# trifectatechfoundation/zlib-rs

Hardware: NVIDIA H100
Metric: deflate_level6_raw_input_throughput_silesia_small_tar (higher is better)
Workload: dtype u8

## Files before the change

### __graft_entry__.py

```python
import os
import subprocess
import sys

ROOT = os.path.dirname(os.path.abspath(__file__))
if ROOT not in sys.path:
    sys.path.insert(0, ROOT)
sys.path.insert(0, os.path.join(ROOT, "tests"))


def build():
    subprocess.check_call(["make", "-C", os.path.join(ROOT, "zlib_rs_b200", "csrc"), "-j8"])
    subprocess.check_call(["make", "-C", os.path.join(ROOT, "oracle")])
    subprocess.check_call(["make", "-C", os.path.join(ROOT, "oracle"), "ref"])
    subprocess.check_call(["make", "-C", os.path.join(ROOT, "tests", "hostmodel")])
    subprocess.check_call(["make", "-C", os.path.join(ROOT, "tests", "skipmodel")])
    subprocess.check_call(["make", "-C", os.path.join(ROOT, "tests", "shardmodel")])
    subprocess.check_call(["make", "-C", os.path.join(ROOT, "tests", "membermodel")])
    subprocess.check_call(["make", "-C", os.path.join(ROOT, "tests", "bgzfmodel")])
    subprocess.check_call(["make", "-C", os.path.join(ROOT, "tests", "batchmodel")])
    subprocess.check_call(["make", "-C", os.path.join(ROOT, "tests", "batchdictmodel")])
    subprocess.check_call(["make", "-C", os.path.join(ROOT, "tests", "batchdictsmodel")])
    subprocess.check_call(["make", "-C", os.path.join(ROOT, "tests", "batchparammodel")])
    subprocess.check_call(["make", "-C", os.path.join(ROOT, "tests", "indexmodel")])
    subprocess.check_call(["make", "-C", os.path.join(ROOT, "tests", "writerindexmodel")])
    subprocess.check_call(["make", "-C", os.path.join(ROOT, "tests", "flushmodel")])
    subprocess.check_call(["make", "-C", os.path.join(ROOT, "tests", "bgzfindexmodel")])
    subprocess.check_call(["make", "-C", os.path.join(ROOT, "tests", "c_client")])
    import zlib_rs_b200
    zlib_rs_b200.lib()


def smoke():
    import zlib
    import zlib_rs_b200 as Z
    import oracle_lib as O
    from corpus import synthetic_mix
    d = synthetic_mix(300000, seed=1)
    out = Z.compress2(d, 6)
    assert out == O.compress(d, 6)[1], "GPU deflate differs from the oracle"
    assert zlib.decompress(out) == d
    assert Z.uncompress(out, len(d)) == d
    assert Z.crc32(d) == O.crc32(d) and Z.adler32(d) == O.adler32(d)
    print("smoke ok: %d -> %d bytes, bit-exact vs oracle" % (len(d), len(out)))


if __name__ == "__main__":
    build()
    if len(sys.argv) > 1 and sys.argv[1] == "smoke":
        smoke()
```

### zlib_rs_b200/csrc/zb_huff.h

```cpp
#pragma once
#include "zb_core.h"

namespace zb {

constexpr int kLCodes = 286, kDCodes = 30, kBlCodes = 19, kHeapSize = 2 * kLCodes + 1;
constexpr int kMaxBits = 15, kMaxBlBits = 7, kEndBlock = 256;
constexpr uint32_t kHdrBytes = 640;

struct HuffTables {
    uint8_t length_code[256];
    uint8_t dist_code[512];
    uint16_t base_length[29];
    uint16_t base_dist[30];
    uint16_t sl_code[288];
    uint8_t sl_len[288];
    uint16_t sd_code[30];
};

ZB_HD uint32_t extra_lbits(uint32_t c) { return (c < 8 || c == 28) ? 0 : (c - 4) >> 2; }
ZB_HD uint32_t extra_dbits(uint32_t c) { return c < 4 ? 0 : (c - 2) >> 1; }
ZB_HD uint32_t extra_blbits(uint32_t c) { return c == 16 ? 2 : c == 17 ? 3 : c == 18 ? 7 : 0; }
ZB_HD uint32_t bl_order(uint32_t i)
{
    return i < 3 ? 16 + i : (i & 1) ? (i == 3 ? 0 : 8 - (i - 3) / 2) : 8 + (i - 4) / 2;
}
ZB_HD uint32_t bit_reverse(uint32_t code, int len)
{
    uint32_t r = 0;
    for (int i = 0; i < len; i++) { r = (r << 1) | (code & 1); code >>= 1; }
    return r;
}
ZB_HD uint32_t d_code(const HuffTables &t, uint32_t dist) { return t.dist_code[dist < 256 ? dist : 256 + (dist >> 7)]; }

ZB_HDN inline void init_tables(HuffTables &t)
{
    int length = 0, dist = 0, code;
    for (code = 0; code < 28; code++) {
        t.base_length[code] = (uint16_t)length;
        for (int n = 0; n < (1 << extra_lbits(code)); n++) t.length_code[length++] = (uint8_t)code;
    }
    t.length_code[length - 1] = 28;
    t.base_length[28] = 0;
    for (code = 0; code < 16; code++) {
        t.base_dist[code] = (uint16_t)dist;
        for (int n = 0; n < (1 << extra_dbits(code)); n++) t.dist_code[dist++] = (uint8_t)code;
    }
    dist >>= 7;
    for (; code < kDCodes; code++) {
        t.base_dist[code] = (uint16_t)(dist << 7);
        for (int n = 0; n < (1 << (extra_dbits(code) - 7)); n++) t.dist_code[256 + dist++] = (uint8_t)code;
    }
    uint16_t next_code[16];
    uint16_t bl_count[16] = {0};
    for (int n = 0; n < 288; n++) {
        t.sl_len[n] = n <= 143 ? 8 : n <= 255 ? 9 : n <= 279 ? 7 : 8;
        bl_count[t.sl_len[n]]++;
    }
    uint32_t c = 0;
    next_code[0] = 0;
    for (int b = 1; b <= 15; b++) { c = (c + bl_count[b - 1]) << 1; next_code[b] = (uint16_t)c; }
    for (int n = 0; n < 288; n++) t.sl_code[n] = (uint16_t)bit_reverse(next_code[t.sl_len[n]]++, t.sl_len[n]);
    for (int n = 0; n < kDCodes; n++) t.sd_code[n] = (uint16_t)bit_reverse((uint32_t)n, 5);
}

struct CtData { uint16_t fc, dl; };

struct TreeScratch {
    CtData ltree[kHeapSize], dtree[2 * kDCodes + 1], bltree[2 * kBlCodes + 1];
    uint32_t heap[kHeapSize];
    uint8_t depth[kHeapSize];
    uint64_t hk[kHeapSize];
};

struct TreeState { uint64_t opt_len, static_len; };

ZB_HD uint32_t freq_depth(const CtData *tree, const uint8_t *depth, uint32_t i) { return ((uint32_t)tree[i].fc << 8) | depth[i]; }

ZB_HDN inline void pqdownheap(TreeScratch &s, int heap_len, int k)
{
    const uint64_t v = s.hk[k], v_val = v >> 16;
    int j = k << 1;
    while (j <= heap_len) {
        uint64_t e = s.hk[j];
        if (j < heap_len) {
            const uint64_t e1 = s.hk[j + 1];
            if ((e1 >> 16) <= (e >> 16)) { j++; e = e1; }
        }
        if (v_val <= (e >> 16)) break;
        s.hk[k] = e;
        k = j;
        j <<= 1;
    }
    s.hk[k] = v;
}
ZB_HD uint64_t heap_entry(const CtData *tree, const uint8_t *depth, uint32_t node) { return ((uint64_t)freq_depth(tree, depth, node) << 16) | node; }

ZB_HDN inline int build_tree(const HuffTables &t, TreeScratch &s, TreeState &st, CtData *tree, int kind)
{
    const int elems = kind == 0 ? kLCodes : kind == 1 ? kDCodes : kBlCodes;
    const int max_length = kind == 2 ? kMaxBlBits : kMaxBits;
    int heap_len = 0, heap_max = kHeapSize, max_code = -1, n, node;
    for (n = 0; n < elems; n++) {
        if (tree[n].fc != 0) { s.heap[++heap_len] = (uint32_t)(max_code = n); s.depth[n] = 0; }
        else tree[n].dl = 0;
    }
    while (heap_len < 2) {
        node = max_code < 2 ? ++max_code : 0;
        s.heap[++heap_len] = (uint32_t)node;
        tree[node].fc = 1;
        s.depth[node] = 0;
        st.opt_len--;
        if (kind == 0) st.static_len -= t.sl_len[node];
        else if (kind == 1) st.static_len -= 5;
    }
    for (n = 1; n <= heap_len; n++) s.hk[n] = heap_entry(tree, s.depth, s.heap[n]);
    for (n = heap_len / 2; n >= 1; n--) pqdownheap(s, heap_len, n);
    node = elems;
    do {
        n = (int)(s.hk[1] & 0xffffu);
        s.hk[1] = s.hk[heap_len--];
        pqdownheap(s, heap_len, 1);
        int m = (int)(s.hk[1] & 0xffffu);
        s.heap[--heap_max] = (uint32_t)n;
        s.heap[--heap_max] = (uint32_t)m;
        tree[node].fc = (uint16_t)(tree[n].fc + tree[m].fc);
        s.depth[node] = (uint8_t)((s.depth[n] >= s.depth[m] ? s.depth[n] : s.depth[m]) + 1);
        tree[n].dl = tree[m].dl = (uint16_t)node;
        s.hk[1] = heap_entry(tree, s.depth, (uint32_t)node);
        node++;
        pqdownheap(s, heap_len, 1);
    } while (heap_len >= 2);
    s.heap[--heap_max] = (uint32_t)(s.hk[1] & 0xffffu);

    uint16_t bl_count[kMaxBits + 1];
    int bits, h, overflow = 0;
    for (bits = 0; bits <= kMaxBits; bits++) bl_count[bits] = 0;
    tree[s.heap[heap_max]].dl = 0;
    for (h = heap_max + 1; h < kHeapSize; h++) {
        n = (int)s.heap[h];
        bits = tree[tree[n].dl].dl + 1;
        if (bits > max_length) { bits = max_length; overflow++; }
        tree[n].dl = (uint16_t)bits;
        if (n > max_code) continue;
        bl_count[bits]++;
        uint32_t xbits = kind == 0 ? (n >= 257 ? extra_lbits(n - 257) : 0) : kind == 1 ? extra_dbits(n) : extra_blbits(n);
        uint64_t f = tree[n].fc;
        st.opt_len += f * (uint64_t)(bits + xbits);
        if (kind == 0) st.static_len += f * (uint64_t)(t.sl_len[n] + xbits);
        else if (kind == 1) st.static_len += f * (uint64_t)(5 + xbits);
    }
    if (overflow > 0) {
        do {
            bits = max_length - 1;
            while (bl_count[bits] == 0) bits--;
// ... 9 lines not shown
                int m = (int)s.heap[--h];
                if (m > max_code) continue;
                if (tree[m].dl != (uint16_t)bits) {
                    st.opt_len += (uint64_t)bits * tree[m].fc;
                    st.opt_len -= (uint64_t)tree[m].dl * tree[m].fc;
                    tree[m].dl = (uint16_t)bits;
                }
                n--;
            }
        }
    }
    uint16_t next_code[kMaxBits + 1];
    uint32_t code = 0;
    next_code[0] = 0;
    for (bits = 1; bits <= kMaxBits; bits++) { code = (code + bl_count[bits - 1]) << 1; next_code[bits] = (uint16_t)code; }
    for (n = 0; n <= max_code; n++) {
        int len = tree[n].dl;
        if (len == 0) continue;
        tree[n].fc = (uint16_t)bit_reverse(next_code[len]++, len);
    }
    return max_code;
}

ZB_HDN inline void scan_tree(CtData *bltree, CtData *tree, int max_code)
{
    int prevlen = -1, curlen, nextlen = tree[0].dl, count = 0, max_count = 7, min_count = 4;
    if (nextlen == 0) { max_count = 138; min_count = 3; }
    tree[max_code + 1].dl = 0xffff;
    for (int n = 0; n <= max_code; n++) {
        curlen = nextlen;
        nextlen = tree[n + 1].dl;
        if (++count < max_count && curlen == nextlen) continue;
        else if (count < min_count) bltree[curlen].fc += (uint16_t)count;
        else if (curlen != 0) {
            if (curlen != prevlen) bltree[curlen].fc++;
            bltree[16].fc++;
        } else if (count <= 10) bltree[17].fc++;
        else bltree[18].fc++;
        count = 0;
        prevlen = curlen;
        if (nextlen == 0) { max_count = 138; min_count = 3; }
        else if (curlen == nextlen) { max_count = 6; min_count = 3; }
        else { max_count = 7; min_count = 4; }
    }
}

struct BitSink {
    uint8_t *buf;
    uint32_t nbits;
    ZB_HD void put(uint32_t val, uint32_t len)
    {
        for (uint32_t i = 0; i < len; i++, nbits++) {
            if ((nbits & 7) == 0) buf[nbits >> 3] = 0;
            buf[nbits >> 3] |= (uint8_t)(((val >> i) & 1u) << (nbits & 7));
        }
    }
};

ZB_HDN inline void send_tree(BitSink &o, const CtData *bltree, const CtData *tree, int max_code)
{
    int prevlen = -1, curlen, nextlen = tree[0].dl, count = 0, max_count = 7, min_count = 4;
    if (nextlen == 0) { max_count = 138; min_count = 3; }
    for (int n = 0; n <= max_code; n++) {
        curlen = nextlen;
        nextlen = tree[n + 1].dl;
        if (++count < max_count && curlen == nextlen) continue;
        else if (count < min_count) { do { o.put(bltree[curlen].fc, bltree[curlen].dl); } while (--count != 0); }
        else if (curlen != 0) {
            if (curlen != prevlen) { o.put(bltree[curlen].fc, bltree[curlen].dl); count--; }
            o.put(bltree[16].fc, bltree[16].dl);
            o.put((uint32_t)(count - 3), 2);
        } else if (count <= 10) {
            o.put(bltree[17].fc, bltree[17].dl);
            o.put((uint32_t)(count - 3), 3);
        } else {
            o.put(bltree[18].fc, bltree[18].dl);
            o.put((uint32_t)(count - 11), 7);
        }
        count = 0;
        prevlen = curlen;
        if (nextlen == 0) { max_count = 138; min_count = 3; }
        else if (curlen == nextlen) { max_count = 6; min_count = 3; }
        else { max_count = 7; min_count = 4; }
    }
}

struct BlockDesc {
    uint32_t sym_begin, sym_count;
    uint32_t in_start, in_len;
    uint32_t type;
    uint32_t last;
    uint32_t hdr_bits;
    uint32_t data_type;
    uint32_t have_window;
    uint32_t no_eob;
    uint64_t body_bits;
    uint64_t bit_base;
    uint16_t lcode[kLCodes];
    uint8_t llen[kLCodes];
    uint16_t dcode[kDCodes];
    uint8_t dlen[kDCodes];
    uint8_t hdr[kHdrBytes];
};

ZB_HDN inline uint32_t detect_data_type(const uint32_t *lfreq)
{
    uint64_t mask = 0xf3ffc07fULL;
    for (int n = 0; n < 32; n++, mask >>= 1)
        if ((mask & 1) && lfreq[n] != 0) return 0;
    if (lfreq[9] != 0 || lfreq[10] != 0 || lfreq[13] != 0) return 1;
    for (int n = 32; n < 256; n++)
        if (lfreq[n] != 0) return 1;
    return 0;
}

ZB_HDN inline void build_block(const HuffTables &t, TreeScratch &s, BlockDesc &b, const uint32_t *lfreq, const uint32_t *dfreq,
                               bool have_window, bool strategy_fixed)
{
    uint64_t opt_lenb, static_lenb;
    int max_blindex = 0, lmax = 0, dmax = 0;
    TreeState st{0, 0};
    b.data_type = 2;
    b.no_eob = 0;
    if (b.sym_count == 0) {
        opt_lenb = static_lenb = 0;
        st.static_len = 7;
    } else {
        b.data_type = detect_data_type(lfreq);
        for (int n = 0; n < kHeapSize; n++) s.ltree[n] = CtData{(uint16_t)(n < kLCodes ? lfreq[n] : 0), 0};
        s.ltree[kEndBlock].fc = 1;
        for (int n = 0; n < 2 * kDCodes + 1; n++) s.dtree[n] = CtData{(uint16_t)(n < kDCodes ? dfreq[n] : 0), 0};
        for (int n = 0; n < 2 * kBlCodes + 1; n++) s.bltree[n] = CtData{0, 0};
        lmax = build_tree(t, s, st, s.ltree, 0);
        dmax = build_tree(t, s, st, s.dtree, 1);
        scan_tree(s.bltree, s.ltree, lmax);
        scan_tree(s.bltree, s.dtree, dmax);
        build_tree(t, s, st, s.bltree, 2);
        for (max_blindex = kBlCodes - 1; max_blindex >= 3; max_blindex--)
            if (s.bltree[bl_order(max_blindex)].dl != 0) break;
        st.opt_len += 3 * ((uint64_t)max_blindex + 1) + 5 + 5 + 4;
        opt_lenb = (st.opt_len + 3 + 7) >> 3;
        static_lenb = (st.static_len + 3 + 7) >> 3;
        if (static_lenb <= opt_lenb || strategy_fixed) opt_lenb = static_lenb;
    }
    BitSink o{b.hdr, 0};
    if ((uint64_t)b.in_len + 4 <= opt_lenb && have_window) {
        b.type = 0;
        o.put(b.last, 3);
        b.hdr_bits = 3;
        b.body_bits = 0;
    } else if (static_lenb == opt_lenb) {
        b.type = 1;
        o.put(2 | b.last, 3);
        b.hdr_bits = 3;
        b.body_bits = st.static_len;
        for (int n = 0; n < kLCodes; n++) { b.lcode[n] = t.sl_code[n]; b.llen[n] = t.sl_len[n]; }
        for (int n = 0; n < kDCodes; n++) { b.dcode[n] = t.sd_code[n]; b.dlen[n] = 5; }
    } else {
        b.type = 2;
        o.put(4 | b.last, 3);
        int lcodes = lmax + 1, dcodes = dmax + 1, blcodes = max_blindex + 1;
        o.put((uint32_t)(lcodes - 257), 5);
        o.put((uint32_t)(dcodes - 1), 5);
        o.put((uint32_t)(blcodes - 4), 4);
        for (int r = 0; r < blcodes; r++) o.put(s.bltree[bl_order(r)].dl, 3);
        send_tree(o, s.bltree, s.ltree, lcodes - 1);
// ... 53 lines not shown
```

### zlib_rs_b200/csrc/zb_kernels.cu

```cuda
#include "zb_kernels.cuh"

namespace zb {

__constant__ HuffTables c_tab;

cudaError_t upload_tables()
{
    HuffTables t;
    init_tables(t);
    return cudaMemcpyToSymbol(c_tab, &t, sizeof t);
}

struct GAcc {
    const uint8_t *data;
    uint32_t N;
    const uint16_t *L;
    const uint32_t *holes;
    const uint32_t *M;
    uint32_t w = kWSize;
    __device__ __forceinline__ uint32_t byte(uint32_t y) const
    {
        while (y >= N) {
            if (y < 2 * w) return 0;
            y -= w;
        }
        return data[y];
    }
    __device__ __forceinline__ uint32_t link(uint32_t y) const { return y + 4 <= N ? L[y] : 0; }
    __device__ __forceinline__ bool inserted(uint32_t y) const { return !((holes[y >> 5] >> (y & 31)) & 1u); }
    __device__ __forceinline__ Match mlook(uint32_t x) const
    {
        uint32_t v = M[x];
        return Match{v >> 16, x - (v & 0xffffu)};
    }
};

struct SAcc {
    const uint8_t *sdata;
    const uint16_t *sL;
    const uint32_t *sholes;
    uint32_t ws;
    __device__ __forceinline__ uint32_t byte(uint32_t y) const { return sdata[y - ws]; }
    __device__ __forceinline__ uint32_t link(uint32_t y) const { return sL[y - ws]; }
    __device__ __forceinline__ bool inserted(uint32_t y) const
    {
        uint32_t i = y - ws;
        return !((sholes[i >> 5] >> (i & 31)) & 1u);
    }
};

struct SAccR {
    const uint8_t *sdata;
    const uint16_t *sL;
    uint32_t ws;
    __device__ __forceinline__ uint32_t byte(uint32_t y) const { return sdata[y - ws]; }
    __device__ __forceinline__ uint32_t link(uint32_t y) const { const uint32_t v = sL[y - ws]; return v == 0xffffu ? 0u : v; }
    __device__ __forceinline__ bool inserted(uint32_t) const { return true; }
};


__device__ __forceinline__ uint32_t lds_u32(const uint32_t *words, uint32_t byte_idx)
{
    const uint32_t w = byte_idx >> 2;
    return __funnelshift_r(words[w], words[w + 1], (byte_idx & 3u) * 8u);
}

constexpr uint32_t kFirstFlag = 0xffffu;

template <bool kRoll>
__device__ __forceinline__ void links2_body(const JobBufs &jb, uint32_t tile0)
{
    const uint32_t tile = tile0 + blockIdx.x;
    extern __shared__ __align__(16) uint8_t smem[];
    constexpr uint32_t kKeys = kRoll ? 32768u : 65536u;
    uint16_t *head = reinterpret_cast<uint16_t *>(smem);
    uint16_t *lists = reinterpret_cast<uint16_t *>(smem + kKeys * 2);
    uint8_t *sd = smem + kKeys * 2 + kLinkTile * 2;
    uint16_t *run = reinterpret_cast<uint16_t *>(smem + kKeys * 2 + kLinkTile * 2 + kLinkTile + 64);
    __shared__ uint16_t c_base[32], c_total[32];
    const uint32_t *words = reinterpret_cast<const uint32_t *>(sd);
    const uint32_t tid = threadIdx.x, lane = tid & 31, warp = tid >> 5;
    const uint32_t N = jb.N, need = kRoll ? 3u : 4u, cap = kRoll ? jb.wsize - 1u : jb.wsize - kMinLookahead;
    const uint32_t ts = tile * kLinkTile;
// ... 1083 lines not shown
};

__global__ void __launch_bounds__(32) k_tail(JobBufs jb)
{
    __shared__ uint32_t ins[1024];
    if (threadIdx.x != 0) return;
    GAcc a{jb.in, jb.N, jb.L, jb.holes, jb.M, jb.wsize};
    const uint32_t p0 = max(jb.info->tail_entry, jb.start);
    const uint32_t n_mid = jb.info->n_mid_syms;
    uint32_t k = 0;
    Sym *syms = jb.syms + n_mid;
    uint32_t *sb = jb.sym_base;
    if (jb.N - p0 > 1024u * 32u - 64u) { atomicOr(&jb.info->error, 4u); return; }
    auto emit = [&](const Sym &s, uint32_t B) {
        syms[k] = s;
        sb[k] = B;
        k++;
    };
    uint32_t fb;
    if (jb.wsize == kWSize) fb = serial_medium(a, jb.N, p0, ins, 1024u, jb.lp, emit);
    else fb = serial_medium(GAccW{a, jb.wsize}, jb.N, p0, ins, 1024u, jb.lp, emit, DynWin{jb.wsize});
    jb.info->n_syms = n_mid + k;
    jb.info->final_base = fb;
    jb.info->n_blocks = (n_mid + k) / jb.block_syms + 1;
}

__device__ __forceinline__ uint32_t sym_end(const Sym &s) { return s.pos + (s.dist ? (uint32_t)s.lc + 3u : 1u); }

__device__ __forceinline__ void block_hist_body(const Sym *syms, uint32_t begin, uint32_t count, uint32_t *fb)
{
    __shared__ uint32_t lf[kLCodes], df[kDCodes];
    for (uint32_t i = threadIdx.x; i < kLCodes; i += blockDim.x) lf[i] = 0;
    if (threadIdx.x < kDCodes) df[threadIdx.x] = 0;
    __syncthreads();
    for (uint32_t i = threadIdx.x; i < count; i += blockDim.x) {
        const Sym s = syms[begin + i];
        if (s.dist == 0) atomicAdd(&lf[s.lc], 1u);
        else {
            atomicAdd(&lf[257 + c_tab.length_code[s.lc]], 1u);
            atomicAdd(&df[d_code(c_tab, s.dist - 1u)], 1u);
        }
    }
    __syncthreads();
    for (uint32_t i = threadIdx.x; i < kLCodes; i += blockDim.x) fb[i] = lf[i];
    if (threadIdx.x < kDCodes) fb[kLCodes + threadIdx.x] = df[threadIdx.x];
}

__global__ void __launch_bounds__(256) k_block_hist(JobBufs jb, uint32_t *freq )
{
    const uint32_t b = blockIdx.x;
    const uint32_t nsyms = jb.info->n_syms, nblocks = jb.info->n_blocks;
    const uint32_t begin = b * jb.block_syms;
    const uint32_t count = (b + 1 < nblocks) ? jb.block_syms : nsyms - begin;
    block_hist_body(jb.syms, begin, count, freq + b * 320);
    if (threadIdx.x == 0) {
        BlockDesc &bd = jb.blocks[b];
        const bool last = b + 1 == nblocks;
        bd.sym_begin = begin;
        bd.sym_count = count;
        bd.last = last && !jb.not_last;
        const uint32_t start = begin == 0 ? jb.start : sym_end(jb.syms[begin - 1]);
        const uint32_t end = last ? jb.N : sym_end(jb.syms[begin + count - 1]);
        bd.in_start = start;
        bd.in_len = end - start;
        uint32_t Bf;
        if (last) Bf = jb.info->final_base;
        else {
            const uint32_t li = begin + count - 1, n_mid = jb.info->n_mid_syms;
            if (jb.serial_mode) {
                Bf = jb.serial_mode == 2 ? jb.block_base[b] : 0;
            } else if (jb.huffman_only) {
                const uint32_t q = jb.syms[li].pos, w = jb.wsize;
                Bf = q < 2 * w ? 0 : w * (1 + (q - 2 * w) / w);
            } else if (jb.slow_mode == 2) {
                Bf = base_at(jb.syms[li].pos, jb.N, jb.wsize);
            } else if (jb.slow_mode) {
                Bf = base_at(jb.syms[li].pos + 1, jb.N, jb.wsize);
            } else Bf = li < n_mid ? wbase_w(DynWin{jb.wsize}, jb.syms[li].pos) : jb.sym_base[li - n_mid];
        }
        bd.have_window = start >= Bf;
    }
}

__device__ __forceinline__ uint32_t brev_bits(uint32_t code, uint32_t len) { return __brev(code) >> (32u - len); }

template <int KIND>
__device__ __forceinline__ uint32_t xbits_of(uint32_t n) { return KIND == 0 ? (n >= 257 ? extra_lbits(n - 257) : 0u) : KIND == 1 ? extra_dbits(n) : extra_blbits(n); }

template <int KIND>
__device__ int build_tree_warp(TreeScratch &s, TreeState &st, CtData *tree, uint32_t *sh_cnt )
{
    constexpr int elems = KIND == 0 ? kLCodes : KIND == 1 ? kDCodes : kBlCodes;
    constexpr int max_length = KIND == 2 ? kMaxBlBits : kMaxBits;
    const uint32_t lane = threadIdx.x & 31;
    int heap_len = 0, max_code = -1;
    for (int b0 = 0; b0 < elems; b0 += 32) {
        const int n = b0 + (int)lane;
        const bool nz = n < elems && tree[n].fc != 0;
        const uint32_t m = __ballot_sync(0xffffffffu, nz);
        if (nz) { s.heap[heap_len + 1 + __popc(m & ((1u << lane) - 1u))] = (uint32_t)n; s.depth[n] = 0; }
        else if (n < elems) tree[n].dl = 0;
        heap_len += __popc(m);
        if (m) max_code = b0 + 31 - __clz(m);
    }
    __syncwarp();
    if (heap_len < 2) {
        if (lane == 0) {
            while (heap_len < 2) {
                const int node = max_code < 2 ? ++max_code : 0;
                s.heap[++heap_len] = (uint32_t)node;
                tree[node].fc = 1;
                s.depth[node] = 0;
                st.opt_len--;
                if (KIND == 0) st.static_len -= c_tab.sl_len[node];
                else if (KIND == 1) st.static_len -= 5;
            }
        }
        heap_len = 2;
        max_code = __shfl_sync(0xffffffffu, max_code, 0);
        __syncwarp();
    }
    for (int n = 1 + (int)lane; n <= heap_len; n += 32) s.hk[n] = heap_entry(tree, s.depth, s.heap[n]);
    __syncwarp();
    for (int lvl = 31 - __clz(heap_len / 2); lvl >= 0; lvl--) {
        const int first = 1 << lvl, last = min((2 << lvl) - 1, heap_len / 2);
        for (int k = first + (int)lane; k <= last; k += 32) pqdownheap(s, heap_len, k);
        __syncwarp();
    }
    int heap_max = kHeapSize;
    if (lane == 0) {
        int node = elems;
        do {
            const int n = (int)(s.hk[1] & 0xffffu);
            s.hk[1] = s.hk[heap_len--];
            pqdownheap(s, heap_len, 1);
            const int m = (int)(s.hk[1] & 0xffffu);
            s.heap[--heap_max] = (uint32_t)n;
            s.heap[--heap_max] = (uint32_t)m;
            tree[node].fc = (uint16_t)(tree[n].fc + tree[m].fc);
            s.depth[node] = (uint8_t)((s.depth[n] >= s.depth[m] ? s.depth[n] : s.depth[m]) + 1);
            tree[n].dl = tree[m].dl = (uint16_t)node;
            s.hk[1] = heap_entry(tree, s.depth, (uint32_t)node);
            node++;
            pqdownheap(s, heap_len, 1);
        } while (heap_len >= 2);
        s.heap[--heap_max] = (uint32_t)(s.hk[1] & 0xffffu);
        int overflow = 0;
        tree[s.heap[heap_max]].dl = 0;
        for (int h = heap_max + 1; h < kHeapSize; h++) {
            const int n = (int)s.heap[h];
            int bits = tree[tree[n].dl].dl + 1;
            if (bits > max_length) { bits = max_length; overflow++; }
            tree[n].dl = (uint16_t)bits;
        }
        sh_cnt[0] = (uint32_t)overflow;
    }
    heap_max = __shfl_sync(0xffffffffu, heap_max, 0);
    __syncwarp();
    const int overflow = (int)sh_cnt[0];
    __syncwarp();
    if (lane < 16) sh_cnt[lane] = 0;
    __syncwarp();
    uint64_t opt = 0, stat = 0;
    for (int n = (int)lane; n <= max_code; n += 32) {
        const uint32_t bits = tree[n].dl;
        if (tree[n].fc == 0 || bits == 0) continue;
        atomicAdd(&sh_cnt[bits], 1u);
        const uint32_t xb = xbits_of<KIND>((uint32_t)n);
        const uint64_t f = tree[n].fc;
        opt += f * (uint64_t)(bits + xb);
        if (KIND == 0) stat += f * (uint64_t)(c_tab.sl_len[n] + xb);
        else if (KIND == 1) stat += f * (uint64_t)(5 + xb);
    }
#pragma unroll
    for (int d = 16; d >= 1; d >>= 1) { opt += __shfl_xor_sync(0xffffffffu, opt, d); stat += __shfl_xor_sync(0xffffffffu, stat, d); }
    __syncwarp();
    if (lane == 0) {
        st.opt_len += opt;
        st.static_len += stat;
        if (overflow > 0) {
            int ov = overflow, bits;
            do {
                bits = max_length - 1;
                while (sh_cnt[bits] == 0) bits--;
                sh_cnt[bits]--;
                sh_cnt[bits + 1] += 2;
                sh_cnt[max_length]--;
                ov -= 2;
            } while (ov > 0);
            int h = kHeapSize;
            for (bits = max_length; bits != 0; bits--) {
                int n = (int)sh_cnt[bits];
                while (n != 0) {
                    const int m = (int)s.heap[--h];
                    if (m > max_code) continue;
                    if (tree[m].dl != (uint16_t)bits) {
                        st.opt_len += (uint64_t)bits * tree[m].fc;
                        st.opt_len -= (uint64_t)tree[m].dl * tree[m].fc;
                        tree[m].dl = (uint16_t)bits;
                    }
                    n--;
                }
            }
        }
    }
    __syncwarp();
    uint32_t nc = 0;
    {
        uint32_t code = 0;
        for (uint32_t b = 1; b <= (uint32_t)kMaxBits; b++) { code = (code + sh_cnt[b - 1]) << 1; if (b == lane) nc = code; }
    }
    for (int b0 = 0; b0 <= max_code; b0 += 32) {
        const int n = b0 + (int)lane;
        const uint32_t len = n <= max_code ? tree[n].dl : 0u;
        const uint32_t same = __match_any_sync(0xffffffffu, len);
        const uint32_t rank = __popc(same & ((1u << lane) - 1u));
        const uint32_t base = __shfl_sync(0xffffffffu, nc, len & 31u);
        if (len) tree[n].fc = (uint16_t)brev_bits(base + rank, len);
#pragma unroll 1
        for (uint32_t l = 1; l <= (uint32_t)kMaxBits; l++) {
            const uint32_t cnt = __popc(__ballot_sync(0xffffffffu, len == l));
            if (lane == l) nc += cnt;
        }
    }
    __syncwarp();
    return max_code;
}

struct WordSink {
    uint8_t *buf;
    uint32_t nbits;
    __device__ __forceinline__ void put(uint32_t val, uint32_t len)
    {
        const uint32_t byte = nbits >> 3, sh = nbits & 7u;
        const uint32_t v = (val & ((1u << len) - 1u)) << sh;
        if (sh == 0) buf[byte] = (uint8_t)v; else buf[byte] |= (uint8_t)v;
        if (sh + len > 8) { buf[byte + 1] = (uint8_t)(v >> 8); if (sh + len > 16) buf[byte + 2] = (uint8_t)(v >> 16); }
        nbits += len;
    }
};

__device__ void send_tree_fast(WordSink &o, const CtData *bltree, const CtData *tree, int max_code)
{
    int prevlen = -1, curlen, nextlen = tree[0].dl, count = 0, max_count = 7, min_count = 4;
    if (nextlen == 0) { max_count = 138; min_count = 3; }
    for (int n = 0; n <= max_code; n++) {
        curlen = nextlen;
        nextlen = tree[n + 1].dl;
        if (++count < max_count && curlen == nextlen) continue;
        else if (count < min_count) { do { o.put(bltree[curlen].fc, bltree[curlen].dl); } while (--count != 0); }
        else if (curlen != 0) {
            if (curlen != prevlen) { o.put(bltree[curlen].fc, bltree[curlen].dl); count--; }
            o.put(bltree[16].fc, bltree[16].dl);
            o.put((uint32_t)(count - 3), 2);
        } else if (count <= 10) {
            o.put(bltree[17].fc, bltree[17].dl);
            o.put((uint32_t)(count - 3), 3);
        } else {
            o.put(bltree[18].fc, bltree[18].dl);
            o.put((uint32_t)(count - 11), 7);
        }
        count = 0;
        prevlen = curlen;
        if (nextlen == 0) { max_count = 138; min_count = 3; }
        else if (curlen == nextlen) { max_count = 6; min_count = 3; }
        else { max_count = 7; min_count = 4; }
    }
}

__device__ void build_block_warp(TreeScratch &s, BlockDesc &b, const uint32_t *lfreq, const uint32_t *dfreq, bool have_window,
                                 bool strategy_fixed, uint32_t *sh_cnt, TreeState *sh_st)
{
    const uint32_t lane = threadIdx.x & 31;
    uint64_t opt_lenb = 0, static_lenb = 0;
    int max_blindex = 0, lmax = 0, dmax = 0;
    TreeState &st = *sh_st;
    if (lane == 0) { st = TreeState{0, 0}; b.data_type = 2; b.no_eob = 0; }
    __syncwarp();
    if (b.sym_count == 0) {
        if (lane == 0) st.static_len = 7;
    } else {
        {
            bool black = false, white = false;
            for (uint32_t n = lane; n < 256; n += 32) {
                if (lfreq[n] == 0) continue;
                if (n < 32 && ((0xf3ffc07fu >> n) & 1u)) black = true;
                if (n == 9 || n == 10 || n == 13 || n >= 32) white = true;
            }
            const bool ab = __any_sync(0xffffffffu, black), aw = __any_sync(0xffffffffu, white);
            if (lane == 0) b.data_type = ab ? 0u : aw ? 1u : 0u;
        }
        for (int n = (int)lane; n < kHeapSize; n += 32) s.ltree[n] = CtData{(uint16_t)(n < kLCodes ? lfreq[n] : 0), 0};
        for (int n = (int)lane; n < 2 * kDCodes + 1; n += 32) s.dtree[n] = CtData{(uint16_t)(n < kDCodes ? dfreq[n] : 0), 0};
        for (int n = (int)lane; n < 2 * kBlCodes + 1; n += 32) s.bltree[n] = CtData{0, 0};
        __syncwarp();
        if (lane == 0) s.ltree[kEndBlock].fc = 1;
        __syncwarp();
        lmax = build_tree_warp<0>(s, st, s.ltree, sh_cnt);
        dmax = build_tree_warp<1>(s, st, s.dtree, sh_cnt);
        if (lane == 0) {
            scan_tree(s.bltree, s.ltree, lmax);
            scan_tree(s.bltree, s.dtree, dmax);
        }
        __syncwarp();
        build_tree_warp<2>(s, st, s.bltree, sh_cnt);
        for (max_blindex = kBlCodes - 1; max_blindex >= 3; max_blindex--)
            if (s.bltree[bl_order(max_blindex)].dl != 0) break;
        if (lane == 0) st.opt_len += 3 * ((uint64_t)max_blindex + 1) + 5 + 5 + 4;
        __syncwarp();
        opt_lenb = (st.opt_len + 3 + 7) >> 3;
        static_lenb = (st.static_len + 3 + 7) >> 3;
        if (static_lenb <= opt_lenb || strategy_fixed) opt_lenb = static_lenb;
    }
    __syncwarp();
    if ((uint64_t)b.in_len + 4 <= opt_lenb && have_window) {
        if (lane == 0) { b.type = 0; b.hdr[0] = (uint8_t)b.last; b.hdr_bits = 3; b.body_bits = 0; }
    } else if (static_lenb == opt_lenb) {
        if (lane == 0) { b.type = 1; b.hdr[0] = (uint8_t)(2 | b.last); b.hdr_bits = 3; b.body_bits = st.static_len; }
        for (int n = (int)lane; n < kLCodes; n += 32) { b.lcode[n] = c_tab.sl_code[n]; b.llen[n] = c_tab.sl_len[n]; }
        if (lane < (uint32_t)kDCodes) { b.dcode[lane] = c_tab.sd_code[lane]; b.dlen[lane] = 5; }
    } else {
        if (lane == 0) {
            b.type = 2;
            WordSink o{b.hdr, 0};
            o.put(4 | b.last, 3);
            const int lcodes = lmax + 1, dcodes = dmax + 1, blcodes = max_blindex + 1;
            o.put((uint32_t)(lcodes - 257), 5);
            o.put((uint32_t)(dcodes - 1), 5);
            o.put((uint32_t)(blcodes - 4), 4);
            for (int r = 0; r < blcodes; r++) o.put(s.bltree[bl_order(r)].dl, 3);
            send_tree_fast(o, s.bltree, s.ltree, lcodes - 1);
            send_tree_fast(o, s.bltree, s.dtree, dcodes - 1);
            b.hdr_bits = o.nbits;
            b.body_bits = 3 + st.opt_len - o.nbits;
        }
        for (int n = (int)lane; n < kLCodes; n += 32) { b.lcode[n] = n <= lmax ? s.ltree[n].fc : 0; b.llen[n] = n <= lmax ? (uint8_t)s.ltree[n].dl : 0; }
        if (lane < (uint32_t)kDCodes) { b.dcode[lane] = (int)lane <= dmax ? s.dtree[lane].fc : 0; b.dlen[lane] = (int)lane <= dmax ? (uint8_t)s.dtree[lane].dl : 0; }
    }
    __syncwarp();
}

__device__ __forceinline__ void build_blocks_body(BlockDesc *gbd, const uint32_t *fb, bool quick, bool first, bool last_piece,
                                                  bool final_block, bool strategy_fixed)
{
    __shared__ TreeScratch s;
    __shared__ BlockDesc bd;
    __shared__ uint32_t fr[320];
    __shared__ uint32_t sh_cnt[16];
    __shared__ TreeState sh_st;
    for (uint32_t i = threadIdx.x; i < 320; i += 32) fr[i] = fb[i];
    for (uint32_t i = threadIdx.x; i < sizeof(BlockDesc) / 4; i += 32)
        reinterpret_cast<uint32_t *>(&bd)[i] = reinterpret_cast<const uint32_t *>(gbd)[i];
    __syncwarp();
    if (quick) {
        if (threadIdx.x == 0) build_quick_piece(c_tab, bd, fr, fr + kLCodes, first, last_piece, final_block);
    } else build_block_warp(s, bd, fr, fr + kLCodes, bd.have_window != 0, strategy_fixed, sh_cnt, &sh_st);
    __syncwarp();
    for (uint32_t i = threadIdx.x; i < sizeof(BlockDesc) / 4; i += 32)
        reinterpret_cast<uint32_t *>(gbd)[i] = reinterpret_cast<const uint32_t *>(&bd)[i];
}

__global__ void __launch_bounds__(32) k_build_blocks(JobBufs jb, const uint32_t *freq)
{
    const uint32_t b = blockIdx.x;
    if (b >= jb.info->n_blocks) return;
    build_blocks_body(&jb.blocks[b], freq + b * 320, jb.serial_mode == 1, b == 0, b + 1 == jb.info->n_blocks, jb.not_last == 0,
                      jb.strategy_fixed != 0);
}

__device__ __forceinline__ void or_bits(uint32_t *out32, uint64_t pos, uint64_t val, uint32_t n)
{
    if (n == 0) return;
    const uint64_t w = pos >> 5;
    const uint32_t sh = (uint32_t)(pos & 31);
    atomicOr(&out32[w], (uint32_t)(val << sh));
    if (sh + n > 32) {
        atomicOr(&out32[w + 1], (uint32_t)(val >> (32 - sh)));
        if (sh + n > 64) atomicOr(&out32[w + 2], (uint32_t)(val >> (64 - sh)));
    }
}

constexpr uint32_t kScanChunk = 1024;
__global__ void __launch_bounds__(256) k_scan_blocks(JobBufs jb)
{
    __shared__ uint64_t s_bits[kScanChunk];
    __shared__ uint64_t s_base[kScanChunk];
    __shared__ uint64_t s_bit;
    const uint32_t nb = jb.info->n_blocks;
    if (threadIdx.x == 0) s_bit = 8ull * jb.hdr_len + jb.prime_bits;
    for (uint32_t c0 = 0; c0 < nb; c0 += kScanChunk) {
        const uint32_t nc = min(kScanChunk, nb - c0);
        for (uint32_t i = threadIdx.x; i < nc; i += blockDim.x) {
            const BlockDesc &bd = jb.blocks[c0 + i];
            s_bits[i] = bd.type == 0 ? (1ull << 63) | (uint16_t)bd.in_len : (uint64_t)bd.hdr_bits + bd.body_bits;
        }
        __syncthreads();
        if (threadIdx.x == 0) {
            uint64_t bit = s_bit;
            for (uint32_t i = 0; i < nc; i++) {
                s_base[i] = bit;
                const uint64_t v = s_bits[i];
                bit = (v >> 63) ? ((bit + 3 + 7) & ~7ull) + 32 + 8ull * (v & 0xffffu) : bit + v;
            }
            s_bit = bit;
        }
        __syncthreads();
        for (uint32_t i = threadIdx.x; i < nc; i += blockDim.x) jb.blocks[c0 + i].bit_base = s_base[i];
        __syncthreads();
    }
    if (threadIdx.x != 0) return;
    uint64_t bit = s_bit;
    if (jb.not_last && jb.end_mode == 0) {
        const uint64_t p = (bit + 3 + 7) & ~7ull;
        jb.info->marker_byte = p >> 3;
        bit = p + 32;
    } else if (jb.not_last && jb.end_mode == 1) {
        or_bits(reinterpret_cast<uint32_t *>(jb.out), bit, 2u, 10);
        bit += 10;
    }
    jb.info->total_bits = bit;
    const uint64_t bytes = (jb.not_last && jb.end_mode ? (bit >> 3) : ((bit + 7) >> 3)) + (jb.wrap == 1 ? 4 : jb.wrap == 2 ? 8 : 0);
    jb.info->out_bytes = bytes;
    jb.info->data_type = jb.blocks[0].sym_count ? jb.blocks[0].data_type : 2u;
    if (bytes > jb.out_cap) { atomicOr(&jb.info->error, 8u); return; }
    stream_header(jb.out, jb.wrap, zlib_level_flags(jb.level, jb.huffman_only || jb.strategy_fixed), jb.cinfo, jb.xfl);
}

__device__ __forceinline__ void encode_body(const BlockDesc &bd, const Sym *syms, const uint8_t *in, uint8_t *out, uint32_t *error)
{
    __shared__ HuffTables st;
    __shared__ uint16_t s_lcode[kLCodes], s_dcode[kDCodes];
    __shared__ uint8_t s_llen[kLCodes], s_dlen[kDCodes];
    __shared__ uint64_t warp_sum[32];
    uint32_t *out32 = reinterpret_cast<uint32_t *>(out);
    const uint32_t tid = threadIdx.x;
    if (bd.type == 0) {
        const uint64_t p = ((bd.bit_base + 3 + 7) >> 3);
        const uint32_t sl = (uint16_t)bd.in_len;
        if (tid == 0) {
            or_bits(out32, bd.bit_base, bd.hdr[0] & 7u, 3);
            out[p] = (uint8_t)sl;
            out[p + 1] = (uint8_t)(sl >> 8);
// ... 308 lines not shown
```

Baseline: 1.648.

## Parallelize Huffman tree construction and header emission across the warp

Replaces the single-lane heap build with packed 32-bit or 64-bit heap keys and a vectorized sift-down. Bit lengths are now computed by a warp-parallel pointer-jumping pass instead of a serial walk. The run-length scan and tree header emission become warp-parallel, using ballot-found runs, a prefix sum of bit counts and atomicOr writes into a zeroed header. The goal is to shorten the serial latency of the per-block tree-building kernel, at the cost of extra shared memory, more synchronisation and new bit-exactness risks. Optional clock64 stamps for profiling are added behind a compile flag.

```diff
diff --git a/__graft_entry__.py b/__graft_entry__.py
--- a/__graft_entry__.py
+++ b/__graft_entry__.py
@@ -25,6 +25,7 @@
     subprocess.check_call(["make", "-C", os.path.join(ROOT, "tests", "writerindexmodel")])
     subprocess.check_call(["make", "-C", os.path.join(ROOT, "tests", "flushmodel")])
     subprocess.check_call(["make", "-C", os.path.join(ROOT, "tests", "bgzfindexmodel")])
+    subprocess.check_call(["make", "-C", os.path.join(ROOT, "tests", "huffmodel")])
     subprocess.check_call(["make", "-C", os.path.join(ROOT, "tests", "c_client")])
     import zlib_rs_b200
     zlib_rs_b200.lib()
diff --git a/zlib_rs_b200/csrc/zb_huff.h b/zlib_rs_b200/csrc/zb_huff.h
--- a/zlib_rs_b200/csrc/zb_huff.h
+++ b/zlib_rs_b200/csrc/zb_huff.h
@@ -69,7 +69,7 @@
     CtData ltree[kHeapSize], dtree[2 * kDCodes + 1], bltree[2 * kBlCodes + 1];
     uint32_t heap[kHeapSize];
     uint8_t depth[kHeapSize];
-    uint64_t hk[kHeapSize];
+    alignas(16) uint64_t hk[kHeapSize + 3];
 };
 
 struct TreeState { uint64_t opt_len, static_len; };
@@ -245,6 +245,25 @@
         if (nextlen == 0) { max_count = 138; min_count = 3; }
         else if (curlen == nextlen) { max_count = 6; min_count = 3; }
         else { max_count = 7; min_count = 4; }
+    }
+}
+
+template <class Emit>
+ZB_HDN inline void run_codes(uint32_t v, uint32_t len, Emit &&emit)
+{
+    uint32_t max_count = v == 0 ? 138u : 7u, min_count = v == 0 ? 3u : 4u;
+    bool first = true;
+    while (len) {
+        uint32_t count = len < max_count ? len : max_count;
+        len -= count;
+        if (count < min_count) { do emit(v, 0u, 0u); while (--count != 0); }
+        else if (v != 0) {
+            if (first) { emit(v, 0u, 0u); count--; }
+            emit(16u, count - 3, 2u);
+        } else if (count <= 10) emit(17u, count - 3, 3u);
+        else emit(18u, count - 11, 7u);
+        first = false;
+        if (v != 0) { max_count = 6; min_count = 3; }
     }
 }
 
diff --git a/zlib_rs_b200/csrc/zb_kernels.cu b/zlib_rs_b200/csrc/zb_kernels.cu
--- a/zlib_rs_b200/csrc/zb_kernels.cu
+++ b/zlib_rs_b200/csrc/zb_kernels.cu
@@ -1,4 +1,5 @@
 #include "zb_kernels.cuh"
+#include <cstdio>
 
 namespace zb {
 
@@ -1248,10 +1249,136 @@
     }
 }
 
+#ifdef ZB_BUILD_CYCLES
+__shared__ long long zb_stamp[12];
+#define ZB_STAMP(i) do { if ((threadIdx.x & 31) == 0) zb_stamp[i] = clock64(); } while (0)
+#else
+#define ZB_STAMP(i) do { } while (0)
+#endif
+
 __device__ __forceinline__ uint32_t brev_bits(uint32_t code, uint32_t len) { return __brev(code) >> (32u - len); }
 
 template <int KIND>
 __device__ __forceinline__ uint32_t xbits_of(uint32_t n) { return KIND == 0 ? (n >= 257 ? extra_lbits(n - 257) : 0u) : KIND == 1 ? extra_dbits(n) : extra_blbits(n); }
+
+template <typename T, int NB, int DB>
+struct HeapKey {
+    using type = T;
+    static constexpr int nb = NB, fb = NB + DB;
+    static constexpr T node_mask = (T(1) << NB) - 1, depth_mask = (T(1) << DB) - 1;
+    __device__ __forceinline__ static T make(uint32_t freq, uint32_t depth, uint32_t node) { return ((T)freq << (NB + DB)) | ((T)depth << NB) | node; }
+};
+using Key32 = HeapKey<uint32_t, 10, 5>;
+using Key64 = HeapKey<unsigned long long, 16, 8>;
+constexpr uint32_t kKey32MaxTotal = 1u << 17;
+
+template <typename T> struct Vec2;
+template <> struct Vec2<uint32_t> { using type = uint2; };
+template <> struct Vec2<unsigned long long> { using type = ulonglong2; };
+
+template <typename K, typename T = typename K::type>
+__device__ __forceinline__ void sift_down(T *h, int heap_len, int k, T v)
+{
+    using V = typename Vec2<T>::type;
+    constexpr int NB = K::nb;
+    const T vv = v >> NB;
+    int j = k << 1;
+    V c = *reinterpret_cast<const V *>(h + j);
+    while (j <= heap_len) {
+        const V g0 = reinterpret_cast<const V *>(h + 2 * j)[0], g1 = reinterpret_cast<const V *>(h + 2 * j)[1];
+        const bool right = j < heap_len && (c.y >> NB) <= (c.x >> NB);
+        const T e = right ? c.y : c.x;
+        if (vv <= (e >> NB)) break;
+        h[k] = e;
+        k = j + (int)right;
+        c = right ? g1 : g0;
+        j = k << 1;
+    }
+    h[k] = v;
+}
+
+template <typename K, typename T = typename K::type>
+__device__ int heap_build_warp(TreeScratch &s, CtData *tree, int heap_len, int node)
+{
+    constexpr int NB = K::nb, FB = K::fb;
+    const uint32_t lane = threadIdx.x & 31;
+    T *h = reinterpret_cast<T *>(s.hk);
+    for (int n = 1 + (int)lane; n <= heap_len; n += 32) { const uint32_t v = s.heap[n]; h[n] = K::make(tree[v].fc, 0, v); }
+    __syncwarp();
+    for (int lvl = 31 - __clz(heap_len / 2); lvl >= 0; lvl--) {
+        const int first = 1 << lvl, last = min((2 << lvl) - 1, heap_len / 2);
+        for (int k = first + (int)lane; k <= last; k += 32) sift_down<K>(h, heap_len, k, h[k]);
+        __syncwarp();
+    }
+    int heap_max = kHeapSize;
+    if (lane == 0) {
+        do {
+            const T kn = h[1];
+            sift_down<K>(h, heap_len - 1, 1, h[heap_len]);
+            heap_len--;
+            const T km = h[1];
+            const uint32_t n = (uint32_t)(kn & K::node_mask), m = (uint32_t)(km & K::node_mask);
+            s.heap[--heap_max] = n;
+            s.heap[--heap_max] = m;
+            const uint32_t f = (uint16_t)((uint32_t)(kn >> FB) + (uint32_t)(km >> FB));
+            const uint32_t dn = (uint32_t)((kn >> NB) & K::depth_mask), dm = (uint32_t)((km >> NB) & K::depth_mask);
+            tree[node].fc = (uint16_t)f;
+            tree[n].dl = tree[m].dl = (uint16_t)node;
+            sift_down<K>(h, heap_len, 1, K::make(f, (max(dn, dm) + 1) & (uint32_t)K::depth_mask, (uint32_t)node));
+            node++;
+        } while (heap_len >= 2);
+        s.heap[--heap_max] = (uint32_t)(h[1] & K::node_mask);
+    }
+    __syncwarp();
+    return __shfl_sync(0xffffffffu, heap_max, 0);
+}
+
+template <int MAX_LENGTH>
+__device__ int tree_lengths_warp(TreeScratch &s, CtData *tree, int heap_max)
+{
+    constexpr int kPer = (kHeapSize + 31) / 32;
+    const uint32_t lane = threadIdx.x & 31;
+    uint32_t *A = reinterpret_cast<uint32_t *>(s.hk), *B = A + kHeapSize + 3;
+    const uint32_t root = s.heap[heap_max];
+    uint32_t nd[kPer];
+#pragma unroll
+    for (int i = 0; i < kPer; i++) {
+        const int h = heap_max + (int)lane + 32 * i;
+        nd[i] = h < kHeapSize ? s.heap[h] : 0xffffu;
+        if (nd[i] != 0xffffu) A[nd[i]] = nd[i] == root ? root << 16 : ((uint32_t)tree[nd[i]].dl << 16) | 1u;
+    }
+    __syncwarp();
+    for (;;) {
+        bool more = false;
+#pragma unroll
+        for (int i = 0; i < kPer; i++) {
+            if (nd[i] == 0xffffu) continue;
+            uint32_t w = A[nd[i]];
+            const uint32_t p = w >> 16;
+            if (p != root) {
+                const uint32_t wp = A[p];
+                w = (wp & 0xffff0000u) | ((w & 0xffffu) + (wp & 0xffffu));
+                more |= (w >> 16) != root;
+            }
+            B[nd[i]] = w;
+        }
+        __syncwarp();
+        uint32_t *t = A; A = B; B = t;
+        if (!__any_sync(0xffffffffu, more)) break;
+    }
+    int overflow = 0;
+#pragma unroll
+    for (int i = 0; i < kPer; i++) {
+        if (nd[i] == 0xffffu) continue;
+        const int depth = (int)(A[nd[i]] & 0xffffu);
+        overflow += depth > MAX_LENGTH;
+        tree[nd[i]].dl = (uint16_t)min(depth, MAX_LENGTH);
+    }
+#pragma unroll
+    for (int d = 16; d >= 1; d >>= 1) overflow += __shfl_xor_sync(0xffffffffu, overflow, d);
+    __syncwarp();
+    return overflow;
+}
 
 template <int KIND>
 __device__ int build_tree_warp(TreeScratch &s, TreeState &st, CtData *tree, uint32_t *sh_cnt )
@@ -1260,11 +1387,12 @@
     constexpr int max_length = KIND == 2 ? kMaxBlBits : kMaxBits;
     const uint32_t lane = threadIdx.x & 31;
     int heap_len = 0, max_code = -1;
+    uint32_t total = 0;
     for (int b0 = 0; b0 < elems; b0 += 32) {
         const int n = b0 + (int)lane;
         const bool nz = n < elems && tree[n].fc != 0;
         const uint32_t m = __ballot_sync(0xffffffffu, nz);
-        if (nz) { s.heap[heap_len + 1 + __popc(m & ((1u << lane) - 1u))] = (uint32_t)n; s.depth[n] = 0; }
+        if (nz) { s.heap[heap_len + 1 + __popc(m & ((1u << lane) - 1u))] = (uint32_t)n; total += tree[n].fc; }
         else if (n < elems) tree[n].dl = 0;
         heap_len += __popc(m);
         if (m) max_code = b0 + 31 - __clz(m);
@@ -1276,7 +1404,7 @@
                 const int node = max_code < 2 ? ++max_code : 0;
                 s.heap[++heap_len] = (uint32_t)node;
                 tree[node].fc = 1;
-                s.depth[node] = 0;
+                total++;
                 st.opt_len--;
                 if (KIND == 0) st.static_len -= c_tab.sl_len[node];
                 else if (KIND == 1) st.static_len -= 5;
@@ -1286,45 +1414,14 @@
         max_code = __shfl_sync(0xffffffffu, max_code, 0);
         __syncwarp();
     }
-    for (int n = 1 + (int)lane; n <= heap_len; n += 32) s.hk[n] = heap_entry(tree, s.depth, s.heap[n]);
-    __syncwarp();
-    for (int lvl = 31 - __clz(heap_len / 2); lvl >= 0; lvl--) {
-        const int first = 1 << lvl, last = min((2 << lvl) - 1, heap_len / 2);
-        for (int k = first + (int)lane; k <= last; k += 32) pqdownheap(s, heap_len, k);
-        __syncwarp();
-    }
-    int heap_max = kHeapSize;
-    if (lane == 0) {
-        int node = elems;
-        do {
-            const int n = (int)(s.hk[1] & 0xffffu);
-            s.hk[1] = s.hk[heap_len--];
-            pqdownheap(s, heap_len, 1);
-            const int m = (int)(s.hk[1] & 0xffffu);
-            s.heap[--heap_max] = (uint32_t)n;
-            s.heap[--heap_max] = (uint32_t)m;
-            tree[node].fc = (uint16_t)(tree[n].fc + tree[m].fc);
-            s.depth[node] = (uint8_t)((s.depth[n] >= s.depth[m] ? s.depth[n] : s.depth[m]) + 1);
-            tree[n].dl = tree[m].dl = (uint16_t)node;
-            s.hk[1] = heap_entry(tree, s.depth, (uint32_t)node);
-            node++;
-            pqdownheap(s, heap_len, 1);
-        } while (heap_len >= 2);
-        s.heap[--heap_max] = (uint32_t)(s.hk[1] & 0xffffu);
-        int overflow = 0;
-        tree[s.heap[heap_max]].dl = 0;
-        for (int h = heap_max + 1; h < kHeapSize; h++) {
-            const int n = (int)s.heap[h];
-            int bits = tree[tree[n].dl].dl + 1;
-            if (bits > max_length) { bits = max_length; overflow++; }
-            tree[n].dl = (uint16_t)bits;
-        }
-        sh_cnt[0] = (uint32_t)overflow;
-    }
-    heap_max = __shfl_sync(0xffffffffu, heap_max, 0);
-    __syncwarp();
-    const int overflow = (int)sh_cnt[0];
-    __syncwarp();
+#pragma unroll
+    for (int d = 16; d >= 1; d >>= 1) total += __shfl_xor_sync(0xffffffffu, total, d);
+    if (KIND == 0) ZB_STAMP(2);
+    const int heap_max = total < kKey32MaxTotal ? heap_build_warp<Key32>(s, tree, heap_len, elems)
+                                                : heap_build_warp<Key64>(s, tree, heap_len, elems);
+    if (KIND == 0) ZB_STAMP(3);
+    const int overflow = tree_lengths_warp<max_length>(s, tree, heap_max);
+    if (KIND == 0) ZB_STAMP(4);
     if (lane < 16) sh_cnt[lane] = 0;
     __syncwarp();
     uint64_t opt = 0, stat = 0;
@@ -1406,37 +1503,83 @@
     }
 };
 
-__device__ void send_tree_fast(WordSink &o, const CtData *bltree, const CtData *tree, int max_code)
-{
-    int prevlen = -1, curlen, nextlen = tree[0].dl, count = 0, max_count = 7, min_count = 4;
-    if (nextlen == 0) { max_count = 138; min_count = 3; }
-    for (int n = 0; n <= max_code; n++) {
-        curlen = nextlen;
-        nextlen = tree[n + 1].dl;
-        if (++count < max_count && curlen == nextlen) continue;
-        else if (count < min_count) { do { o.put(bltree[curlen].fc, bltree[curlen].dl); } while (--count != 0); }
-        else if (curlen != 0) {
-            if (curlen != prevlen) { o.put(bltree[curlen].fc, bltree[curlen].dl); count--; }
-            o.put(bltree[16].fc, bltree[16].dl);
-            o.put((uint32_t)(count - 3), 2);
-        } else if (count <= 10) {
-            o.put(bltree[17].fc, bltree[17].dl);
-            o.put((uint32_t)(count - 3), 3);
-        } else {
-            o.put(bltree[18].fc, bltree[18].dl);
-            o.put((uint32_t)(count - 11), 7);
-        }
-        count = 0;
-        prevlen = curlen;
-        if (nextlen == 0) { max_count = 138; min_count = 3; }
-        else if (curlen == nextlen) { max_count = 6; min_count = 3; }
-        else { max_count = 7; min_count = 4; }
-    }
+constexpr int kRunWords = (kLCodes + kDCodes + 1 + 31) / 32;
+
+__device__ __forceinline__ uint32_t code_len_at(const TreeScratch &s, int i, int lcodes) { return i < lcodes ? s.ltree[i].dl : s.dtree[i - lcodes].dl; }
+
+__device__ __forceinline__ void find_runs(const TreeScratch &s, int lcodes, int dcodes, uint32_t *starts)
+{
+    const int lane = (int)(threadIdx.x & 31), total = lcodes + dcodes;
+    for (int w = 0; w < kRunWords; w++) {
+        const int i = 32 * w + lane;
+        const bool st = i <= total && (i == 0 || i == lcodes || i == total || code_len_at(s, i, lcodes) != code_len_at(s, i - 1, lcodes));
+        const uint32_t m = __ballot_sync(0xffffffffu, st);
+        if (lane == 0) starts[w] = m;
+    }
+    __syncwarp();
+}
+
+__device__ __forceinline__ uint32_t run_length(const uint32_t *starts, int i)
+{
+    int w = i >> 5;
+    uint32_t m = starts[w] & ~((2u << (i & 31)) - 1u);
+    while (m == 0) m = starts[++w];
+    return (uint32_t)(32 * w + __ffs(m) - 1 - i);
+}
+
+__device__ void scan_trees_warp(const TreeScratch &s, CtData *bltree, int lcodes, int dcodes, uint32_t *starts, uint32_t *cnt )
+{
+    const int lane = (int)(threadIdx.x & 31);
+    if (lane < kBlCodes) cnt[lane] = 0;
+    find_runs(s, lcodes, dcodes, starts);
+    for (int w = 0; w < kRunWords; w++) {
+        const int i = 32 * w + lane;
+        if (i < lcodes + dcodes && ((starts[w] >> lane) & 1u))
+            run_codes(code_len_at(s, i, lcodes), run_length(starts, i), [&](uint32_t sym, uint32_t, uint32_t) { atomicAdd(&cnt[sym], 1u); });
+    }
+    __syncwarp();
+    if (lane < kBlCodes) bltree[lane].fc = (uint16_t)cnt[lane];
+    __syncwarp();
+}
+
+__device__ uint32_t send_trees_warp(const TreeScratch &s, const CtData *bltree, int lcodes, int dcodes, const uint32_t *starts,
+                                    uint32_t *hdr, uint32_t bit)
+{
+    const uint32_t lane = threadIdx.x & 31;
+    auto put = [&](uint32_t &pos, uint32_t val, uint32_t len) {
+        if (len == 0) return;
+        const uint32_t v = val & ((1u << len) - 1u), sh = pos & 31u;
+        atomicOr(&hdr[pos >> 5], v << sh);
+        if (sh + len > 32) atomicOr(&hdr[(pos >> 5) + 1], v >> (32 - sh));
+        pos += len;
+    };
+    for (int w = 0; w < kRunWords; w++) {
+        const int i = 32 * w + (int)lane;
+        const bool st = i < lcodes + dcodes && ((starts[w] >> lane) & 1u);
+        uint32_t v = 0, len = 0, nb = 0;
+        if (st) {
+            v = code_len_at(s, i, lcodes);
+            len = run_length(starts, i);
+            run_codes(v, len, [&](uint32_t sym, uint32_t, uint32_t xb) { nb += bltree[sym].dl + xb; });
+        }
+        uint32_t incl = nb;
+#pragma unroll
+        for (int k = 1; k < 32; k <<= 1) { const uint32_t t = __shfl_up_sync(0xffffffffu, incl, k); if (lane >= (uint32_t)k) incl += t; }
+        if (st) {
+            uint32_t pos = bit + incl - nb;
+            run_codes(v, len, [&](uint32_t sym, uint32_t extra, uint32_t xb) { put(pos, bltree[sym].fc, bltree[sym].dl); put(pos, extra, xb); });
+        }
+        bit += __shfl_sync(0xffffffffu, incl, 31);
+    }
+    __syncwarp();
+    return bit;
 }
 
 __device__ void build_block_warp(TreeScratch &s, BlockDesc &b, const uint32_t *lfreq, const uint32_t *dfreq, bool have_window,
                                  bool strategy_fixed, uint32_t *sh_cnt, TreeState *sh_st)
 {
+    static_assert(offsetof(BlockDesc, hdr) % 4 == 0 && kHdrBytes % 4 == 0, "the header is written in 32-bit words");
+    __shared__ uint32_t sh_runs[kRunWords];
     const uint32_t lane = threadIdx.x & 31;
     uint64_t opt_lenb = 0, static_lenb = 0;
     int max_blindex = 0, lmax = 0, dmax = 0;
@@ -1463,13 +1606,13 @@
         if (lane == 0) s.ltree[kEndBlock].fc = 1;
         __syncwarp();
         lmax = build_tree_warp<0>(s, st, s.ltree, sh_cnt);
+        ZB_STAMP(5);
         dmax = build_tree_warp<1>(s, st, s.dtree, sh_cnt);
-        if (lane == 0) {
-            scan_tree(s.bltree, s.ltree, lmax);
-            scan_tree(s.bltree, s.dtree, dmax);
-        }
-        __syncwarp();
+        ZB_STAMP(6);
+        scan_trees_warp(s, s.bltree, lmax + 1, dmax + 1, sh_runs, sh_cnt);
+        ZB_STAMP(7);
         build_tree_warp<2>(s, st, s.bltree, sh_cnt);
+        ZB_STAMP(8);
         for (max_blindex = kBlCodes - 1; max_blindex >= 3; max_blindex--)
             if (s.bltree[bl_order(max_blindex)].dl != 0) break;
         if (lane == 0) st.opt_len += 3 * ((uint64_t)max_blindex + 1) + 5 + 5 + 4;
@@ -1486,19 +1629,25 @@
         for (int n = (int)lane; n < kLCodes; n += 32) { b.lcode[n] = c_tab.sl_code[n]; b.llen[n] = c_tab.sl_len[n]; }
         if (lane < (uint32_t)kDCodes) { b.dcode[lane] = c_tab.sd_code[lane]; b.dlen[lane] = 5; }
     } else {
+        const int lcodes = lmax + 1, dcodes = dmax + 1, blcodes = max_blindex + 1;
+        uint32_t *hdr = reinterpret_cast<uint32_t *>(b.hdr);
+        for (uint32_t i = lane; i < kHdrBytes / 4; i += 32) hdr[i] = 0;
+        __syncwarp();
         if (lane == 0) {
             b.type = 2;
             WordSink o{b.hdr, 0};
             o.put(4 | b.last, 3);
-            const int lcodes = lmax + 1, dcodes = dmax + 1, blcodes = max_blindex + 1;
             o.put((uint32_t)(lcodes - 257), 5);
             o.put((uint32_t)(dcodes - 1), 5);
             o.put((uint32_t)(blcodes - 4), 4);
             for (int r = 0; r < blcodes; r++) o.put(s.bltree[bl_order(r)].dl, 3);
-            send_tree_fast(o, s.bltree, s.ltree, lcodes - 1);
-            send_tree_fast(o, s.bltree, s.dtree, dcodes - 1);
-            b.hdr_bits = o.nbits;
-            b.body_bits = 3 + st.opt_len - o.nbits;
+        }
+        __syncwarp();
+        const uint32_t nbits = send_trees_warp(s, s.bltree, lcodes, dcodes, sh_runs, hdr, 17u + 3u * (uint32_t)blcodes);
+        ZB_STAMP(9);
+        if (lane == 0) {
+            b.hdr_bits = nbits;
+            b.body_bits = 3 + st.opt_len - nbits;
         }
         for (int n = (int)lane; n < kLCodes; n += 32) { b.lcode[n] = n <= lmax ? s.ltree[n].fc : 0; b.llen[n] = n <= lmax ? (uint8_t)s.ltree[n].dl : 0; }
         if (lane < (uint32_t)kDCodes) { b.dcode[lane] = (int)lane <= dmax ? s.dtree[lane].fc : 0; b.dlen[lane] = (int)lane <= dmax ? (uint8_t)s.dtree[lane].dl : 0; }
@@ -1512,18 +1661,29 @@
     __shared__ TreeScratch s;
     __shared__ BlockDesc bd;
     __shared__ uint32_t fr[320];
-    __shared__ uint32_t sh_cnt[16];
+    __shared__ uint32_t sh_cnt[32];
     __shared__ TreeState sh_st;
+    ZB_STAMP(0);
     for (uint32_t i = threadIdx.x; i < 320; i += 32) fr[i] = fb[i];
     for (uint32_t i = threadIdx.x; i < sizeof(BlockDesc) / 4; i += 32)
         reinterpret_cast<uint32_t *>(&bd)[i] = reinterpret_cast<const uint32_t *>(gbd)[i];
     __syncwarp();
+    ZB_STAMP(1);
     if (quick) {
         if (threadIdx.x == 0) build_quick_piece(c_tab, bd, fr, fr + kLCodes, first, last_piece, final_block);
     } else build_block_warp(s, bd, fr, fr + kLCodes, bd.have_window != 0, strategy_fixed, sh_cnt, &sh_st);
     __syncwarp();
     for (uint32_t i = threadIdx.x; i < sizeof(BlockDesc) / 4; i += 32)
         reinterpret_cast<uint32_t *>(gbd)[i] = reinterpret_cast<const uint32_t *>(&bd)[i];
+#ifdef ZB_BUILD_CYCLES
+    ZB_STAMP(10);
+    if (threadIdx.x == 0 && !quick) {
+        long long d[10];
+        for (int i = 0; i < 10; i++) d[i] = zb_stamp[i + 1] - zb_stamp[0];
+        ::printf("build_cycles %u: %lld %lld %lld %lld %lld %lld %lld %lld %lld %lld\n", blockIdx.x, d[0], d[1], d[2], d[3], d[4], d[5],
+               d[6], d[7], d[8], d[9]);
+    }
+#endif
 }
 
 __global__ void __launch_bounds__(32) k_build_blocks(JobBufs jb, const uint32_t *freq)
```

Result: faster. 1.682 (median of 6 runs) (+2.1%).
